# burn-research/OpenMEASURE

Measured on AMD Instinct MI355X. Metric: SPR fit+reconstruct throughput (GB/s snapshot matrix), higher is better.
Workload: dtype f64

## Files before the change

openmeasure_amd/csrc/common.hpp:

```cpp
#pragma once
#include <hip/hip_runtime.h>
#include <stdint.h>
#include <stdio.h>

#include "spr_hip.h"

typedef double f64x4 __attribute__((ext_vector_type(4)));
typedef double f64x2 __attribute__((ext_vector_type(2)));

void spr_set_error(const char *fmt, ...);

#define SPR_REQUIRE(cond, code, ...)      \
  do {                                    \
    if (!(cond)) {                        \
      spr_set_error(__VA_ARGS__);         \
      return (code);                      \
    }                                     \
  } while (0)

#define SPR_HIP_TRY(expr)                                                          \
  do {                                                                             \
    hipError_t e__ = (expr);                                                       \
    if (e__ != hipSuccess) {                                                       \
      spr_set_error("%s failed: %s (%s:%d)", #expr, hipGetErrorString(e__),       \
                    __FILE__, __LINE__);                                           \
      return SPR_E_HIP;                                                            \
    }                                                                              \
  } while (0)

#define SPR_LAUNCH_CHECK()                                                         \
  do {                                                                             \
    hipError_t e__ = hipGetLastError();                                            \
    if (e__ != hipSuccess) {                                                       \
      spr_set_error("kernel launch failed: %s (%s:%d)", hipGetErrorString(e__),   \
                    __FILE__, __LINE__);                                           \
      return SPR_E_HIP;                                                            \
    }                                                                              \
  } while (0)

int spr_cached_cus();

struct SegPlan {
  int64_t row0, n_rows, n_points;
  int32_t n_features;
  int32_t total_wg;
  int32_t chunk_rows;
};

__host__ __device__ inline void seg_range(const SegPlan &p, int f, int64_t &lo, int64_t &hi) {
  int64_t glo = (int64_t)f * p.n_points, ghi = glo + p.n_points;
  if (glo < p.row0) glo = p.row0;
  if (ghi > p.row0 + p.n_rows) ghi = p.row0 + p.n_rows;
  if (ghi < glo) ghi = glo;
  lo = glo - p.row0;
  hi = ghi - p.row0;
}

__host__ __device__ inline int seg_wgs(const SegPlan &p, int64_t rows) {
  if (rows <= 0) return 0;
  int64_t w = rows * (int64_t)p.total_wg / p.n_rows;
  int64_t chunks = (rows + p.chunk_rows - 1) / p.chunk_rows;
  if (w > chunks) w = chunks;
  if (w < 1) w = 1;
  return (int)w;
}

__host__ __device__ inline int seg_first_feature(const SegPlan &p) { return (int)(p.row0 / p.n_points); }
__host__ __device__ inline int seg_last_feature(const SegPlan &p) {
  int64_t f = (p.row0 + p.n_rows - 1) / p.n_points;
  if (f > p.n_features - 1) f = p.n_features - 1;
  return (int)f;
}

inline int seg_total_wgs(const SegPlan &p) {
  int tot = 0;
  for (int f = seg_first_feature(p); f <= seg_last_feature(p); ++f) {
    int64_t lo, hi;
    seg_range(p, f, lo, hi);
    tot += seg_wgs(p, hi - lo);
  }
  return tot;
}

__device__ inline bool seg_locate(const SegPlan &p, int b, int &f, int &wl, int &wpf, int &base,
                                  int64_t &lo, int64_t &hi) {
  int acc = 0;
  int f1 = seg_last_feature(p);
  for (int ff = seg_first_feature(p); ff <= f1; ++ff) {
    seg_range(p, ff, lo, hi);
    int w = seg_wgs(p, hi - lo);
    if (b < acc + w) {
      f = ff; wl = b - acc; wpf = w; base = acc;
      return true;
    }
    acc += w;
  }
  return false;
}

template <int CTRL>
__device__ inline double dpp_f64(double v) {
  union { double d; int i[2]; } a, b;
  a.d = v;
  b.i[0] = __builtin_amdgcn_update_dpp(0, a.i[0], CTRL, 0xF, 0xF, true);
  b.i[1] = __builtin_amdgcn_update_dpp(0, a.i[1], CTRL, 0xF, 0xF, true);
  return b.d;
}

template <int WIDTH>
__device__ inline double group_sum_t(double v) {
  if (WIDTH >= 2) v += dpp_f64<0xB1>(v);
  if (WIDTH >= 4) v += dpp_f64<0x4E>(v);
  if (WIDTH >= 8) v += dpp_f64<0x141>(v);
  if (WIDTH >= 16) v += dpp_f64<0x140>(v);
  if (WIDTH >= 32) v += __shfl_xor(v, 16, 64);
  if (WIDTH >= 64) v += __shfl_xor(v, 32, 64);
  return v;
}

__device__ inline double group_sum(double v, int width) {
  for (int o = width >> 1; o > 0; o >>= 1) v += __shfl_xor(v, o, 64);
  return v;
}

constexpr int spr_pow2_divisor_le64(int n) {
  int p = 1;
  while (p < 64 && n % (2 * p) == 0) p *= 2;
  return p;
}

inline int spr_round_mt(int m) {
  static const int sup[] = {1, 2, 3, 4, 6, 8, 12, 16};
  int need = (m + 15) / 16;
  for (int s : sup)
    if (s >= need) return s;
  return -1;
}
```

openmeasure_amd/csrc/field_dot.hpp:

```cpp
#pragma once
#include "common.hpp"

constexpr int SPR_FIELD_NF = 1;

template <int NT>
__device__ inline double field_row_value(const double (&v)[NT], const double (&a)[NT], double scale, double mean) {
  double d = 0.0;
#pragma unroll
  for (int ct = 0; ct < NT; ++ct) d = fma(v[ct], a[ct], d);
  return fma(scale, group_sum_t<16>(d), mean);
}
```

openmeasure_amd/csrc/project_ws.hip:

```cpp
#include <type_traits>

#include "rowtile.hpp"
#include "launch.hpp"
#include "project_ws.hpp"
#include "field_dot.hpp"

namespace {

constexpr int WS_WAVES = 8;
constexpr int WS_ROWS = 16 * WS_WAVES;

template <int RT> struct WsLds { static constexpr int NC = 16 * RT, LDW = NC; static_assert(RT % 2 == 0, "column tiles come in pairs"); };

template <typename TX> struct WsPiece;
template <> struct WsPiece<double> { f64x2 a, b; };
template <> struct WsPiece<float> { float x, y, z, w; };

template <int VEC, typename TX>
__device__ inline WsPiece<TX> ws_load(const TX *__restrict__ rp, int col0, int m) {
  WsPiece<TX> p;
  if constexpr (std::is_same<TX, double>::value) {
    if (VEC) {
      p.a = *reinterpret_cast<const f64x2 *>(rp + col0);
      p.b = *reinterpret_cast<const f64x2 *>(rp + col0 + 2);
    } else {
      p.a.x = rp[col0 < m ? col0 : 0];         p.a.y = rp[col0 + 1 < m ? col0 + 1 : 0];
      p.b.x = rp[col0 + 2 < m ? col0 + 2 : 0]; p.b.y = rp[col0 + 3 < m ? col0 + 3 : 0];
    }
  } else {
    if (VEC) {
      const float4 v = *reinterpret_cast<const float4 *>(rp + col0);
      p.x = v.x; p.y = v.y; p.z = v.z; p.w = v.w;
    } else {
      p.x = rp[col0 < m ? col0 : 0];         p.y = rp[col0 + 1 < m ? col0 + 1 : 0];
      p.z = rp[col0 + 2 < m ? col0 + 2 : 0]; p.w = rp[col0 + 3 < m ? col0 + 3 : 0];
    }
  }
  return p;
}

template <typename TX>
__device__ inline double ws_elem(const WsPiece<TX> &p, int t) {
  if constexpr (std::is_same<TX, double>::value) return t == 0 ? p.a.x : t == 1 ? p.a.y : t == 2 ? p.b.x : p.b.y;
  else return (double)(t == 0 ? p.x : t == 1 ? p.y : t == 2 ? p.z : p.w);
}

template <int MT, int RT, int VEC, typename TX, typename TU, bool NRM, int NF>
__global__ __launch_bounds__(WS_WAVES * 64) void project_ws_kernel(
    const TX *__restrict__ X, int64_t ldx, int m, int center_i, SegPlan plan, const double *__restrict__ inv_scale,
    const double *__restrict__ rowmean, const double *__restrict__ W, int r, TU *__restrict__ Ur, int64_t ldu,
    double *__restrict__ nrm2, WsField fld) {
  constexpr int K = 16 * MT, NJ = MT;
  constexpr int NC = WsLds<RT>::NC, LDW = WsLds<RT>::LDW;
  __shared__ double Wl[K * LDW];

  int f, wl, wpf, base;
  int64_t lo, hi;
  if (!seg_locate(plan, blockIdx.x, f, wl, wpf, base, lo, hi)) return;

  const int lane = threadIdx.x & 63;
  const int wave = __builtin_amdgcn_readfirstlane(threadIdx.x >> 6);
  const int li = lane & 15, kk = lane >> 4;
  const double isc = inv_scale[f];

  for (int e = threadIdx.x; e < K * NC; e += WS_WAVES * 64) {
    const int k = e / NC, c = e - k * NC;
    Wl[k * LDW + (c >> 5) * 32 + (c & 15) * 2 + ((c >> 4) & 1)] = (k < m && c < r) ? W[(int64_t)k * r + c] * isc : 0.0;
  }
  __syncthreads();
  double wbar[RT];
#pragma unroll
  for (int ct = 0; ct < RT; ++ct) {
    double sacc = 0.0;
    if (center_i != 0) {
      for (int k = kk; k < K; k += 4) sacc += Wl[k * LDW + (ct >> 1) * 32 + li * 2 + (ct & 1)];
      sacc += __shfl_xor(sacc, 16, 64);
      sacc += __shfl_xor(sacc, 32, 64);
    }
    wbar[ct] = sacc;
  }

  double av[NF > 0 ? NF : 1][RT];
  double fsc = 0.0;
  if constexpr (NF > 0) {
    fsc = fld.scale[f];
#pragma unroll
    for (int v = 0; v < NF; ++v)
#pragma unroll
      for (int ct = 0; ct < RT; ++ct)
        av[v][ct] = (v < fld.n_p && 16 * ct + li < r) ? fld.A[(int64_t)v * r + 16 * ct + li] : 0.0;
  }

  const int64_t nchunks = (hi - lo + WS_ROWS - 1) / WS_ROWS;
  int64_t c = wl;
  if (c >= nchunks) return;
  const double *wb = Wl + (4 * kk) * LDW + 2 * li;
  const double *wb_hi = wb + 128 * LDW;

  auto row_ptr = [&](int64_t cc) {
    int64_t row = lo + cc * WS_ROWS + 16 * wave + li;
    row = row < hi ? row : hi - 1;
    return X + row * ldx;
  };
  WsPiece<TX> areg[NJ];
  {
    const TX *rp = row_ptr(c);
#pragma unroll
    for (int j = 0; j < NJ; ++j) areg[j] = ws_load<VEC, TX>(rp, 16 * j + 4 * kk, m);
  }
  while (c < nchunks) {
    const int64_t cn = c + wpf;
    const TX *rpn = row_ptr(cn < nchunks ? cn : c);
    const int64_t blk0 = lo + c * WS_ROWS + 16 * wave;
    double mu[4];
#pragma unroll
    for (int i = 0; i < 4; ++i) {
      const int64_t rr = blk0 + kk + 4 * i;
      const double v = rowmean[rr < hi ? rr : hi - 1];
      mu[i] = center_i != 0 ? v : 0.0;
    }
    f64x4 acc[RT];
#pragma unroll
    for (int ct = 0; ct < RT; ++ct) acc[ct] = (f64x4){0.0, 0.0, 0.0, 0.0};
    f64x2 bcur[RT / 2], bnxt[RT / 2];
#pragma unroll
    for (int p = 0; p < RT / 2; ++p) bcur[p] = *reinterpret_cast<const f64x2 *>(wb + 32 * p);
#pragma unroll
    for (int j = 0; j < NJ; ++j) {
#pragma unroll
      for (int t = 0; t < 4; ++t) {
        const int sn = 4 * j + t + 1;
        const int jn = (sn >> 2) % NJ, tn = sn & 3;
        const double *wj = (jn < 8 ? wb : wb_hi) + (16 * (jn & 7) + tn) * LDW;
#pragma unroll
        for (int p = 0; p < RT / 2; ++p) bnxt[p] = *reinterpret_cast<const f64x2 *>(wj + 32 * p);
        const double a = ws_elem<TX>(areg[j], t);
#pragma unroll
        for (int p = 0; p < RT / 2; ++p) {
          acc[2 * p] = __builtin_amdgcn_mfma_f64_16x16x4f64(a, bcur[p].x, acc[2 * p], 0, 0, 0);
          acc[2 * p + 1] = __builtin_amdgcn_mfma_f64_16x16x4f64(a, bcur[p].y, acc[2 * p + 1], 0, 0, 0);
        }
        if (t == 3) areg[j] = ws_load<VEC, TX>(rpn, 16 * j + 4 * kk, m);
        __builtin_amdgcn_sched_group_barrier(0x100, RT / 2, 0);
        __builtin_amdgcn_sched_group_barrier(0x008, RT, 0);
        __builtin_amdgcn_sched_barrier(0);
#pragma unroll
        for (int p = 0; p < RT / 2; ++p) bcur[p] = bnxt[p];
      }
    }
    {
      const bool full = (blk0 + 16 <= hi) && (r == NC);
      TU *up = Ur + (blk0 + kk) * ldu + li;
      double q[4] = {0.0, 0.0, 0.0, 0.0};
      double sv[NF > 0 ? 4 : 1][RT];
#pragma unroll
      for (int ct = 0; ct < RT; ++ct) {
        const double s[4] = {acc[ct].x - mu[0] * wbar[ct], acc[ct].y - mu[1] * wbar[ct],
                             acc[ct].z - mu[2] * wbar[ct], acc[ct].w - mu[3] * wbar[ct]};
        if (NRM) {
#pragma unroll
          for (int i = 0; i < 4; ++i) { const double v = (double)(TU)s[i]; q[i] = fma(v, v, q[i]); }
        }
        if constexpr (NF > 0) {
#pragma unroll
          for (int i = 0; i < 4; ++i) sv[i][ct] = (double)(TU)s[i];
        }
        if (full) {
#pragma unroll
          for (int i = 0; i < 4; ++i) up[4 * i * ldu + 16 * ct] = (TU)s[i];
        } else if (16 * ct + li < r) {
#pragma unroll
          for (int i = 0; i < 4; ++i)
            if (blk0 + kk + 4 * i < hi) up[4 * i * ldu + 16 * ct] = (TU)s[i];
        }
      }
      if (NRM) {
#pragma unroll
        for (int i = 0; i < 4; ++i) {
          const double t = group_sum_t<16>(q[i]);
          if (li == i && blk0 + kk + 4 * i < hi) nrm2[blk0 + kk + 4 * i] = t;
        }
      }
      if constexpr (NF > 0) {
#pragma unroll
        for (int v = 0; v < NF; ++v)
#pragma unroll
          for (int i = 0; i < 4; ++i) {
            const double x = field_row_value<RT>(sv[i], av[v], fsc, mu[i]);
            if (li == i && v < fld.n_p && blk0 + kk + 4 * i < hi) fld.out[(int64_t)v * fld.ldo + blk0 + kk + 4 * i] = x;
          }
      }
    }
    c = cn;
  }
}

template <int MT, int RT, typename TX, typename TU>
int ws_launch(const TX *X, int64_t n_rows, int32_t m, int64_t ldx, int64_t row0, int64_t n_points, int32_t n_features,
              int center, const double *inv_scale, const double *rowmean, const double *W, int32_t r, TU *Ur,
              int64_t ldu, int accumulate, double *nrm2, hipStream_t st, const WsField *field) {
  SegPlan plan = spr_make_plan(row0, n_rows, n_points, n_features, WS_ROWS);
  constexpr int narrow_per_cu = 2;
  const int grid = spr_plan_grid(plan, MT <= 4 ? narrow_per_cu : 1);
  const bool vec = (m == 16 * MT) && spr_rows_aligned16(X, sizeof(TX) * ldx);
  if (!vec) return SPR_E_UNSUPPORTED;
  const WsField fld = field ? *field : WsField{nullptr, nullptr, 0, nullptr, 0};
#define WS_GO(NRMV, NFV)                                                                                                       \
  hipLaunchKernelGGL((project_ws_kernel<MT, RT, 1, TX, TU, NRMV, NFV>), dim3(grid), dim3(WS_WAVES * 64), 0, st, X, ldx, (int)m, \
                     center, plan, inv_scale, rowmean, W, (int)r, Ur, ldu, nrm2, fld)
  if (field) {
    if (nrm2) WS_GO(true, SPR_FIELD_NF);
    else WS_GO(false, SPR_FIELD_NF);
  } else {
    if (nrm2) WS_GO(true, 0);
    else WS_GO(false, 0);
  }
#undef WS_GO
  SPR_LAUNCH_CHECK();
  return SPR_OK;
}

}


template <typename TX, typename TU>
int spr_project_ws(const TX *d_X, int64_t n_rows, int32_t m, int64_t ldx, int64_t row0, int64_t n_points,
                   int32_t n_features, int32_t center, const double *d_inv_scale, const double *d_rowmean,
                   const double *d_W, int32_t r, TU *d_Ur, int64_t ldu, int32_t accumulate, double *d_rownorm2,
                   hipStream_t st, const WsField *field) {
  if (accumulate) return SPR_E_UNSUPPORTED;
  if (field && (field->n_p < 1 || field->n_p > SPR_FIELD_NF || r % 16 != 0 || !center)) return SPR_E_UNSUPPORTED;
  const int mt = spr_round_mt(m);
  const int need = (r + 15) / 16;
  const int rt = need <= 2 ? 2 : need <= 4 ? 4 : 0;
#define WS(MTV, RTV)                                                                                             \
  if (mt == MTV && rt == RTV)                                                                                    \
    return ws_launch<MTV, RTV, TX, TU>(d_X, n_rows, m, ldx, row0, n_points, n_features, center, d_inv_scale,   \
                                        d_rowmean, d_W, r, d_Ur, ldu, accumulate, d_rownorm2, st, field)
  WS(4, 2); WS(4, 4); WS(8, 2); WS(8, 4); WS(12, 2); WS(12, 4); WS(16, 2); WS(16, 4);
#undef WS
  return SPR_E_UNSUPPORTED;
}

template int spr_project_ws<double, double>(const double *, int64_t, int32_t, int64_t, int64_t, int64_t, int32_t, int32_t,
                                            const double *, const double *, const double *, int32_t, double *, int64_t,
                                            int32_t, double *, hipStream_t, const WsField *);
template int spr_project_ws<float, float>(const float *, int64_t, int32_t, int64_t, int64_t, int64_t, int32_t, int32_t,
                                          const double *, const double *, const double *, int32_t, float *, int64_t,
                                          int32_t, double *, hipStream_t, const WsField *);
template int spr_project_ws<float, double>(const float *, int64_t, int32_t, int64_t, int64_t, int64_t, int32_t, int32_t,
                                           const double *, const double *, const double *, int32_t, double *, int64_t,
                                           int32_t, double *, hipStream_t, const WsField *);
```

openmeasure_amd/csrc/rowtile.hpp:

```cpp
#pragma once
#include "common.hpp"

typedef float f32x2 __attribute__((ext_vector_type(2)));
template <typename TX> struct PieceOf;
template <> struct PieceOf<double> { using type = f64x2; };
template <> struct PieceOf<float> { using type = f32x2; };
__device__ inline f64x2 widen(f64x2 p) { return p; }
__device__ inline f64x2 widen(f32x2 p) { return (f64x2){(double)p.x, (double)p.y}; }

struct RowStats {
  double cnt, ref, s1, s2;
  __device__ inline void init() { cnt = 0.0; ref = 0.0; s1 = 0.0; s2 = 0.0; }
  __device__ inline void push(double x, bool valid) {
    ref = (cnt == 0.0) ? x : ref;
    const double d = valid ? x - ref : 0.0;
    cnt += valid ? 1.0 : 0.0;
    s1 += d;
    s2 += d * d;
  }
  __device__ inline double mean() const { return cnt > 0.0 ? ref + s1 / cnt : 0.0; }
  __device__ inline double m2() const {
    const double v = cnt > 0.0 ? s2 - s1 * s1 / cnt : 0.0;
    return v > 0.0 ? v : 0.0;
  }
// ... 13 lines not shown
  static_assert(R % ROWS_PER_IT == 0, "panel rows must be a multiple of rows per pass");
  static constexpr bool WIDE_STORE = (MP % 2 == 0);

  Piece pre[IT][VPL];
  double pmean[IT];

  template <int VEC>
  __device__ inline void load_pass(int it, const TX *__restrict__ X, int64_t ldx, int m, int64_t crow0,
                                   int64_t seg_hi, int wave, int lane, const double *__restrict__ mean_in = nullptr,
                                   int split = 1 << 30, int64_t gap = 0) {
    const int grp = lane / LPR, lig = lane % LPR;
    int64_t lrow = crow0 + it * ROWS_PER_IT + wave * RPW + grp;
    lrow = lrow < seg_hi ? lrow : seg_hi - 1;
    const TX *rp = X + lrow * ldx;
    if (mean_in) pmean[it] = mean_in[lrow];
#pragma unroll
    for (int v = 0; v < VPL; ++v) {
      const int col = 2 * (lig + v * LPR);
      const int64_t g0 = col >= split ? gap : 0, g1 = col + 1 >= split ? gap : 0;
      Piece t;
      if (VEC == 2) {
        t = *reinterpret_cast<const Piece *>(rp + col + g0);
      } else if (VEC == 1) {
        t = *reinterpret_cast<const Piece *>(rp + (col < m ? col + g0 : 0));
      } else {
        t.x = rp[col < m ? col + g0 : 0];
        t.y = rp[col + 1 < m ? col + 1 + g1 : 0];
      }
      pre[it][v] = t;
    }
  }

  template <int VEC>
  __device__ inline void load_piece(int it, int v, const TX *__restrict__ X, int64_t ldx, int m, int64_t crow0,
                                    int64_t seg_hi, int wave, int lane) {
    const int grp = lane / LPR, lig = lane % LPR;
    int64_t lrow = crow0 + it * ROWS_PER_IT + wave * RPW + grp;
    lrow = lrow < seg_hi ? lrow : seg_hi - 1;
    const TX *rp = X + lrow * ldx;
    const int col = 2 * (lig + v * LPR);
    Piece t;
    if (VEC == 2) {
      t = *reinterpret_cast<const Piece *>(rp + col);
    } else if (VEC == 1) {
      t = *reinterpret_cast<const Piece *>(rp + (col < m ? col : 0));
    } else {
      t.x = rp[col < m ? col : 0];
      t.y = rp[col + 1 < m ? col + 1 : 0];
    }
    pre[it][v] = t;
  }

  __device__ inline void raw_store_piece(int it, int v, double *__restrict__ lds, int m, int64_t crow0,
                                         int64_t seg_hi, int wave, int lane) {
    const int grp = lane / LPR, lig = lane % LPR;
    const int rloc = it * ROWS_PER_IT + wave * RPW + grp;
    const bool rv = crow0 + rloc < seg_hi;
    const int col = 2 * (lig + v * LPR);
    f64x2 c = widen(pre[it][v]);
    c.x = (rv && col < m) ? c.x : 0.0;
    c.y = (rv && col + 1 < m) ? c.y : 0.0;
    if constexpr (WIDE_STORE) {
      *reinterpret_cast<f64x2 *>(lds + rloc * MP + col) = c;
    } else {
      lds[rloc * MP + col] = c.x;
      lds[rloc * MP + col + 1] = c.y;
    }
  }

  template <int VEC>
  __device__ inline void load(const TX *__restrict__ X, int64_t ldx, int m, int64_t crow0, int64_t seg_hi,
                              int wave, int lane, const double *__restrict__ mean_in = nullptr, int split = 1 << 30,
                              int64_t gap = 0) {
#pragma unroll
    for (int it = 0; it < IT; ++it) load_pass<VEC>(it, X, ldx, m, crow0, seg_hi, wave, lane, mean_in, split, gap);
  }

  template <bool WRITE_MEAN>
  __device__ inline void center_store_pass(int it, double *__restrict__ lds, int m, int center, int64_t crow0,
                                           int64_t seg_hi, int wave, int lane, double *__restrict__ rowmean,
                                           RowStats *st, double *__restrict__ rowsum = nullptr) {
    const int grp = lane / LPR, lig = lane % LPR;
    const double inv_m = 1.0 / (double)m;
    const int rloc = it * ROWS_PER_IT + wave * RPW + grp;
    const int64_t lrow = crow0 + rloc;
    const bool rv = lrow < seg_hi;
    const bool fast = (crow0 + (it + 1) * ROWS_PER_IT <= seg_hi) && (m == MPAD);
    if (fast) {
      double mean;
      if constexpr (WRITE_MEAN) {
        double s = 0.0;
#pragma unroll
        for (int v = 0; v < VPL; ++v) { const f64x2 w = widen(pre[it][v]); s += w.x + w.y; }
        s = group_sum_t<LPR>(s);
        mean = center == 2 ? pmean[it] : (center ? s * inv_m : 0.0);
        if (rowsum && center == 2 && lig == 0) rowsum[lrow] = s;
      } else {
        mean = center ? pmean[it] : 0.0;
      }
      if (WRITE_MEAN) {
        if (lig == 0 && center != 2) rowmean[lrow] = mean;
        st->push(mean, center != 2);
      }
#pragma unroll
      for (int v = 0; v < VPL; ++v) {
        const int col = 2 * (lig + v * LPR);
        const f64x2 w = widen(pre[it][v]);
        f64x2 c = {w.x - mean, w.y - mean};
        if constexpr (WIDE_STORE) {
          *reinterpret_cast<f64x2 *>(lds + rloc * MP + col) = c;
        } else {
          lds[rloc * MP + col] = c.x;
          lds[rloc * MP + col + 1] = c.y;
        }
      }
      return;
    }
    double s = 0.0;
#pragma unroll
    for (int v = 0; v < VPL; ++v) {
      const int col = 2 * (lig + v * LPR);
      const f64x2 w = widen(pre[it][v]);
      s += (col < m ? w.x : 0.0) + (col + 1 < m ? w.y : 0.0);
    }
    s = group_sum_t<LPR>(s);
    const double mean = center == 2 ? pmean[it] : (center ? s * inv_m : 0.0);
    if (WRITE_MEAN) {
      if (rv && lig == 0 && center != 2) rowmean[lrow] = mean;
      if (rowsum && center == 2 && rv && lig == 0) rowsum[lrow] = s;
      st->push(mean, rv && center != 2);
    }
#pragma unroll
    for (int v = 0; v < VPL; ++v) {
      const int col = 2 * (lig + v * LPR);
      const f64x2 w = widen(pre[it][v]);
      f64x2 c;
      c.x = (rv && col < m) ? w.x - mean : 0.0;
      c.y = (rv && col + 1 < m) ? w.y - mean : 0.0;
      if constexpr (WIDE_STORE) {
        *reinterpret_cast<f64x2 *>(lds + rloc * MP + col) = c;
      } else {
        lds[rloc * MP + col] = c.x;
        lds[rloc * MP + col + 1] = c.y;
      }
    }
  }

  template <bool EXT>
  __device__ inline void load_pass_own(int it, const TX *__restrict__ ubase, int64_t ldx, int64_t lane_off,
                                       int64_t rows_left, int wave, int lane, const double *__restrict__ mean_in,
                                       int64_t crow0, int split = 1 << 30, int64_t gap = 0) {
    const int grp = lane / LPR, lig = lane % LPR;
    const int64_t lrow = (int64_t)it * ROWS_PER_IT + wave * RPW + grp;
    const int64_t last = rows_left > 0 ? rows_left - 1 : 0;
    const bool in = lrow < rows_left;
    const int64_t off = in ? lane_off + (int64_t)it * ROWS_PER_IT * ldx : last * ldx;
    const TX *rp = ubase + off;
    if (EXT) pmean[it] = mean_in[crow0 + (in ? lrow : last)];
#pragma unroll
    for (int v = 0; v < VPL; ++v) {
      const int col = 2 * (lig + v * LPR);
      pre[it][v] = *reinterpret_cast<const Piece *>(rp + col + (col >= split ? gap : 0));
    }
  }

  template <bool FULL, bool EXT, bool SUMS = false>
  __device__ inline void center_store_own(int it, double *__restrict__ lds, int64_t crow0, int64_t rows_left, int wave,
                                          int lane, double *__restrict__ rowmean, double *__restrict__ rowsum = nullptr) {
    const int grp = lane / LPR, lig = lane % LPR;
    constexpr double inv_m = 1.0 / (double)MPAD;
    const int rloc = it * ROWS_PER_IT + wave * RPW + grp;
    const bool rv = FULL || rloc < rows_left;
    f64x2 w[VPL];
#pragma unroll
    for (int v = 0; v < VPL; ++v) w[v] = widen(pre[it][v]);
    double mean;
    if (EXT) {
      mean = pmean[it];
      if (SUMS) {
        double s = w[0].x + w[0].y;
#pragma unroll
        for (int v = 1; v < VPL; ++v) s += w[v].x + w[v].y;
        s = group_sum_t<LPR>(s);
        if (rv && lig == 0) rowsum[crow0 + rloc] = s;
      }
    } else {
      double s = w[0].x + w[0].y;
#pragma unroll
      for (int v = 1; v < VPL; ++v) s += w[v].x + w[v].y;
      s = group_sum_t<LPR>(s);
      mean = s * inv_m;
      if (rv && lig == 0) rowmean[crow0 + rloc] = mean;
    }
#pragma unroll
    for (int v = 0; v < VPL; ++v) {
      const int col = 2 * (lig + v * LPR);
      f64x2 c = {w[v].x - mean, w[v].y - mean};
      if (!FULL) {
        c.x = rv ? c.x : 0.0;
        c.y = rv ? c.y : 0.0;
      }
      *reinterpret_cast<f64x2 *>(lds + rloc * MP + col) = c;
    }
  }

  __device__ inline void raw_store_pass(int it, double *__restrict__ lds, int m, int64_t crow0, int64_t seg_hi,
                                        int wave, int lane) {
    const int grp = lane / LPR, lig = lane % LPR;
    const int rloc = it * ROWS_PER_IT + wave * RPW + grp;
    const bool rv = crow0 + rloc < seg_hi;
    const bool fast = (crow0 + (it + 1) * ROWS_PER_IT <= seg_hi) && (m == MPAD);
#pragma unroll
    for (int v = 0; v < VPL; ++v) {
      const int col = 2 * (lig + v * LPR);
      f64x2 c = widen(pre[it][v]);
      if (!fast) {
        c.x = (rv && col < m) ? c.x : 0.0;
        c.y = (rv && col + 1 < m) ? c.y : 0.0;
      }
      if constexpr (WIDE_STORE) {
        *reinterpret_cast<f64x2 *>(lds + rloc * MP + col) = c;
      } else {
        lds[rloc * MP + col] = c.x;
        lds[rloc * MP + col + 1] = c.y;
      }
    }
  }

  __device__ inline void raw_store(double *__restrict__ lds, int m, int64_t crow0, int64_t seg_hi, int wave,
                                   int lane) {
#pragma unroll
    for (int it = 0; it < IT; ++it) raw_store_pass(it, lds, m, crow0, seg_hi, wave, lane);
  }

  template <bool WRITE_MEAN>
  __device__ inline void center_store(double *__restrict__ lds, int m, int center, int64_t crow0, int64_t seg_hi,
                                      int wave, int lane, double *__restrict__ rowmean, RowStats *st,
                                      double *__restrict__ rowsum = nullptr) {
#pragma unroll
    for (int it = 0; it < IT; ++it)
      center_store_pass<WRITE_MEAN>(it, lds, m, center, crow0, seg_hi, wave, lane, rowmean, st, rowsum);
  }
};
```

openmeasure_amd/csrc/stats_gram.hip:

```cpp
#include <type_traits>

#include "rowtile.hpp"
#include "launch.hpp"

#define GRAM_MFMA(a, b, c) __builtin_amdgcn_mfma_f64_16x16x4f64((a), (b), (c), 0, 0, 0)

namespace {

template <int MT>
struct GramShape {
  static constexpr int MPAD = 16 * MT;
  static constexpr int MP = MPAD + ((MT % 2 == 0) ? 16 : 0);
  static constexpr int T = MT * (MT + 1) / 2;
  static constexpr int NU = (MT + 1) / 2;
};

template <int MT> struct GramCfg;
template <> struct GramCfg<1>  { static constexpr int NW = 8,  R = 64, KS = 8; static constexpr bool DBUF = true; static constexpr int LPRMAX = 16; };
template <> struct GramCfg<2>  { static constexpr int NW = 8,  R = 32, KS = 8; static constexpr bool DBUF = true; static constexpr int LPRMAX = 16; };
template <> struct GramCfg<3>  { static constexpr int NW = 8,  R = 64, KS = 4; static constexpr bool DBUF = true; static constexpr int LPRMAX = 16; };
template <> struct GramCfg<4>  { static constexpr int NW = 8,  R = 64, KS = 4; static constexpr bool DBUF = true; static constexpr int LPRMAX = 8; };
template <> struct GramCfg<6>  { static constexpr int NW = 12, R = 48, KS = 4; static constexpr bool DBUF = true; static constexpr int LPRMAX = 16; };
template <> struct GramCfg<8>  { static constexpr int NW = 8,  R = 32, KS = 2; static constexpr bool DBUF = true; static constexpr int LPRMAX = 16; };
template <> struct GramCfg<12> { static constexpr int NW = 12, R = 24, KS = 2; static constexpr bool DBUF = false; static constexpr int LPRMAX = 32; };
template <> struct GramCfg<16> { static constexpr int NW = 8,  R = 32, KS = 1; static constexpr bool DBUF = false; static constexpr int LPRMAX = 16; };

template <int MT> struct GramOut { static constexpr int KSO = (GramCfg<MT>::KS >= 4) ? 1 : GramCfg<MT>::KS; };

constexpr int tri_index(int mt, int ti, int tj) { return ti * mt - ti * (ti - 1) / 2 + (tj - ti); }

template <int MT>
__device__ inline void tile_coords(int idx, int &ti, int &tj) {
  ti = 0;
  while (ti < MT - 1 && idx >= MT - ti) { idx -= MT - ti; ++ti; }
  tj = ti + idx;
  if (tj > MT - 1) tj = MT - 1;
}

template <int MT, int U, int VEC, typename TX>
__device__ inline void gram_wave(const TX *__restrict__ X, int64_t ldx, int m, int center,
                                 int64_t lo, int64_t hi, int wl, int wpf, int ks, int wave, int lane,
                                 double *__restrict__ lds0, double *__restrict__ lds1,
                                 double *__restrict__ rowmean, double *__restrict__ stat_part,
                                 double *__restrict__ slab, double *__restrict__ rowsum) {
  using S = GramShape<MT>;
  using C = GramCfg<MT>;
  constexpr int R = C::R, KS = C::KS, NW = C::NW, MP = S::MP, T = S::T;
  constexpr int KROWS = R / KS, KSTEPS = KROWS / 4;
  constexpr int RA = U, RB = MT - 1 - U;
  constexpr int NA = MT - RA;
  constexpr int NB = (RB != RA) ? MT - RB : 0;
  static_assert(KROWS % 4 == 0, "k slice must be a multiple of the MFMA depth");
  using RT = RowTile<MT, R, MP, NW, C::LPRMAX, TX>;

  f64x4 accA[NA];
  f64x4 accB[NB > 0 ? NB : 1];
#pragma unroll
  for (int j = 0; j < NA; ++j) accA[j] = (f64x4){0.0, 0.0, 0.0, 0.0};
#pragma unroll
  for (int j = 0; j < NB; ++j) accB[j] = (f64x4){0.0, 0.0, 0.0, 0.0};

  RowStats st;
  st.init();
  RT tile;

  const int64_t nchunks = (hi - lo + R - 1) / R;
  int64_t c = wl;
  const double *mean_in = rowmean;
  tile.template load<VEC>(X, ldx, m, lo + c * R, hi, wave, lane, mean_in);
  tile.template center_store<true>(lds0, m, center, lo + c * R, hi, wave, lane, rowmean, &st, rowsum);
  int64_t cn = c + wpf;
  int64_t nrow0 = (cn < nchunks) ? lo + cn * R : hi;
  tile.template load<VEC>(X, ldx, m, nrow0, hi, wave, lane, mean_in);
  int buf = 0;
  const int frag = (lane >> 4) * MP + (lane & 15) + ks * KROWS * MP + RA * 16;
  while (c < nchunks) {
    double *cur = buf ? lds1 : lds0;
    double *nxt = buf ? lds0 : lds1;
    const int64_t c2 = cn + wpf;
    const int64_t n2row0 = (c2 < nchunks) ? lo + c2 * R : hi;
    __syncthreads();
    const double *p = cur + frag;
    if constexpr (C::DBUF) {
      double op[2][NA];
#pragma unroll
      for (int j = 0; j < NA; ++j) op[0][j] = p[16 * j];
#pragma unroll
      for (int k = 0; k < KSTEPS; ++k) {
        if (k + 1 < KSTEPS) {
#pragma unroll
          for (int j = 0; j < NA; ++j) op[(k + 1) & 1][j] = p[(k + 1) * 4 * MP + 16 * j];
        }
#pragma unroll
        for (int j = 0; j < NA; ++j)
          accA[j] = GRAM_MFMA(op[k & 1][0], op[k & 1][j], accA[j]);
#pragma unroll
        for (int j = 0; j < NB; ++j)
          accB[j] = GRAM_MFMA(op[k & 1][RB - RA], op[k & 1][RB - RA + j], accB[j]);
#pragma unroll
        for (int it = 0; it < RT::IT; ++it)
          if ((it * KSTEPS) / RT::IT == k) {
            tile.template center_store_pass<true>(it, nxt, m, center, nrow0, hi, wave, lane, rowmean, &st, rowsum);
            tile.template load_pass<VEC>(it, X, ldx, m, n2row0, hi, wave, lane, mean_in);
          }
      }
    } else {
#pragma unroll
      for (int k = 0; k < KSTEPS; ++k) {
        double op[NA];
#pragma unroll
        for (int j = 0; j < NA; ++j) op[j] = p[k * 4 * MP + 16 * j];
#pragma unroll
        for (int j = 0; j < NA; ++j)
          accA[j] = GRAM_MFMA(op[0], op[j], accA[j]);
#pragma unroll
        for (int j = 0; j < NB; ++j)
          accB[j] = GRAM_MFMA(op[RB - RA], op[RB - RA + j], accB[j]);
#pragma unroll
        for (int it = 0; it < RT::IT; ++it)
          if ((it * KSTEPS) / RT::IT == k) {
            tile.template center_store_pass<true>(it, nxt, m, center, nrow0, hi, wave, lane, rowmean, &st, rowsum);
            tile.template load_pass<VEC>(it, X, ldx, m, n2row0, hi, wave, lane, mean_in);
          }
      }
    }
    buf ^= 1;
    c = cn;
    cn = c2;
    nrow0 = n2row0;
  }

  constexpr int KSO = GramOut<MT>::KSO;
  if constexpr (KSO != KS) {
    static_assert((size_t)T * 256 <= (size_t)2 * R * MP, "tile staging must fit the panel buffers");
    double *red = lds0 + lane;
    for (int s = KS - 1; s >= 1; --s) {
      __syncthreads();
      if (ks == s) {
#pragma unroll
        for (int j = 0; j < NA; ++j) {
          double *tp = red + tri_index(MT, RA, RA + j) * 256;
          tp[0] = accA[j].x; tp[64] = accA[j].y; tp[128] = accA[j].z; tp[192] = accA[j].w;
        }
#pragma unroll
        for (int j = 0; j < NB; ++j) {
          double *tp = red + tri_index(MT, RB, RB + j) * 256;
          tp[0] = accB[j].x; tp[64] = accB[j].y; tp[128] = accB[j].z; tp[192] = accB[j].w;
        }
      }
      __syncthreads();
      if (ks == s - 1) {
#pragma unroll
        for (int j = 0; j < NA; ++j) {
          const double *tp = red + tri_index(MT, RA, RA + j) * 256;
          accA[j].x += tp[0]; accA[j].y += tp[64]; accA[j].z += tp[128]; accA[j].w += tp[192];
        }
#pragma unroll
        for (int j = 0; j < NB; ++j) {
          const double *tp = red + tri_index(MT, RB, RB + j) * 256;
          accB[j].x += tp[0]; accB[j].y += tp[64]; accB[j].z += tp[128]; accB[j].w += tp[192];
        }
      }
    }
  }
  if (KSO == KS || ks == 0) {
    double *sp = slab + ((int64_t)blockIdx.x * KSO + (KSO == KS ? ks : 0)) * T * 256 + lane;
#pragma unroll
    for (int j = 0; j < NA; ++j) {
      double *tp = sp + (int64_t)tri_index(MT, RA, RA + j) * 256;
      tp[0] = accA[j].x; tp[64] = accA[j].y; tp[128] = accA[j].z; tp[192] = accA[j].w;
    }
#pragma unroll
    for (int j = 0; j < NB; ++j) {
      double *tp = sp + (int64_t)tri_index(MT, RB, RB + j) * 256;
      tp[0] = accB[j].x; tp[64] = accB[j].y; tp[128] = accB[j].z; tp[192] = accB[j].w;
    }
  }
  if ((lane % RT::LPR) == 0) {
    double *q = stat_part + ((int64_t)blockIdx.x * RT::ROWS_PER_IT + wave * RT::RPW + lane / RT::LPR) * 3;
    q[0] = st.cnt; q[1] = st.mean(); q[2] = st.m2();
  }
}

__device__ inline void chan_merge(double &n, double &mu, double &m2, double nb, double mb, double sb) {
  if (nb > 0.0) {
    const double tot = n + nb, d = mb - mu;
    mu += d * nb / tot;
    m2 += sb + d * d * n * nb / tot;
    n = tot;
  }
}

template <int MT, int U, typename TX, bool EXT, bool SUMS>
__device__ inline void gram_wave_own(const TX *__restrict__ X, int64_t ldx, int64_t lo, int64_t hi, int wl, int wpf, int ks,
                                     int wave, int lane, double *__restrict__ lds0, double *__restrict__ lds1,
                                     double *__restrict__ rowmean, double *__restrict__ slab, double *__restrict__ rowsum) {
  using S = GramShape<MT>;
  using C = GramCfg<MT>;
  constexpr int R = C::R, KS = C::KS, NW = C::NW, MP = S::MP, T = S::T;
  constexpr int KROWS = R / KS, KSTEPS = KROWS / 4;
  constexpr int RA = U, RB = MT - 1 - U;
  constexpr int NA = MT - RA;
  constexpr int NB = (RB != RA) ? MT - RB : 0;
  using RT = RowTile<MT, R, MP, NW, C::LPRMAX, TX>;

  f64x4 accA[NA];
  f64x4 accB[NB > 0 ? NB : 1];
#pragma unroll
  for (int j = 0; j < NA; ++j) accA[j] = (f64x4){0.0, 0.0, 0.0, 0.0};
#pragma unroll
  for (int j = 0; j < NB; ++j) accB[j] = (f64x4){0.0, 0.0, 0.0, 0.0};

  RT tile;
  const int64_t nchunks = (hi - lo + R - 1) / R;
  const int64_t lane_off = (int64_t)(wave * RT::RPW + lane / RT::LPR) * ldx;
  auto base_of = [&](int64_t row0) { return X + row0 * ldx; };
  int64_t c = wl;
  int64_t crow0 = lo + c * R;
#pragma unroll
  for (int it = 0; it < RT::IT; ++it) tile.template load_pass_own<EXT>(it, base_of(crow0), ldx, lane_off, hi - crow0, wave, lane, rowmean, crow0);
  if (crow0 + R <= hi) {
#pragma unroll
    for (int it = 0; it < RT::IT; ++it) tile.template center_store_own<true, EXT, SUMS>(it, lds0, crow0, hi - crow0, wave, lane, rowmean, rowsum);
  } else {
#pragma unroll
    for (int it = 0; it < RT::IT; ++it) tile.template center_store_own<false, EXT, SUMS>(it, lds0, crow0, hi - crow0, wave, lane, rowmean, rowsum);
  }
  int64_t cn = c + wpf;
  int64_t nrow0 = (cn < nchunks) ? lo + cn * R : hi;
#pragma unroll
  for (int it = 0; it < RT::IT; ++it) tile.template load_pass_own<EXT>(it, base_of(nrow0 < hi ? nrow0 : lo), ldx, lane_off, hi - nrow0, wave, lane, rowmean, nrow0 < hi ? nrow0 : lo);
  int buf = 0;
  const int frag = (lane >> 4) * MP + (lane & 15) + ks * KROWS * MP + RA * 16;
  while (c < nchunks) {
    double *cur = buf ? lds1 : lds0;
    double *nxt = buf ? lds0 : lds1;
    const int64_t c2 = cn + wpf;
    const int64_t n2row0 = (c2 < nchunks) ? lo + c2 * R : hi;
    const TX *n2base = base_of(n2row0 < hi ? n2row0 : lo);
    const bool nfull = nrow0 + R <= hi;
    __syncthreads();
    const double *p = cur + frag;
    auto stage = [&](auto full_tag, int k) {
      constexpr bool FULL = decltype(full_tag)::value;
#pragma unroll
      for (int it = 0; it < RT::IT; ++it)
        if ((it * KSTEPS) / RT::IT == k) {
          tile.template center_store_own<FULL, EXT, SUMS>(it, nxt, nrow0, hi - nrow0, wave, lane, rowmean, rowsum);
          tile.template load_pass_own<EXT>(it, n2base, ldx, lane_off, hi - n2row0, wave, lane, rowmean, n2row0 < hi ? n2row0 : lo);
        }
    };
    if constexpr (C::DBUF) {
      double op[2][NA];
#pragma unroll
      for (int j = 0; j < NA; ++j) op[0][j] = p[16 * j];
#pragma unroll
      for (int k = 0; k < KSTEPS; ++k) {
        if (k + 1 < KSTEPS) {
#pragma unroll
          for (int j = 0; j < NA; ++j) op[(k + 1) & 1][j] = p[(k + 1) * 4 * MP + 16 * j];
        }
#pragma unroll
        for (int j = 0; j < NA; ++j) accA[j] = GRAM_MFMA(op[k & 1][0], op[k & 1][j], accA[j]);
#pragma unroll
        for (int j = 0; j < NB; ++j) accB[j] = GRAM_MFMA(op[k & 1][RB - RA], op[k & 1][RB - RA + j], accB[j]);
        if (nfull) stage(std::true_type{}, k); else stage(std::false_type{}, k);
      }
    } else {
#pragma unroll
      for (int k = 0; k < KSTEPS; ++k) {
        double op[NA];
#pragma unroll
        for (int j = 0; j < NA; ++j) op[j] = p[k * 4 * MP + 16 * j];
#pragma unroll
        for (int j = 0; j < NA; ++j) accA[j] = GRAM_MFMA(op[0], op[j], accA[j]);
#pragma unroll
        for (int j = 0; j < NB; ++j) accB[j] = GRAM_MFMA(op[RB - RA], op[RB - RA + j], accB[j]);
        if (nfull) stage(std::true_type{}, k); else stage(std::false_type{}, k);
      }
    }
    buf ^= 1;
    c = cn;
    cn = c2;
    nrow0 = n2row0;
  }
  double *sp = slab + ((int64_t)blockIdx.x * KS + ks) * T * 256 + lane;
#pragma unroll
  for (int j = 0; j < NA; ++j) {
    double *tp = sp + (int64_t)tri_index(MT, RA, RA + j) * 256;
    tp[0] = accA[j].x; tp[64] = accA[j].y; tp[128] = accA[j].z; tp[192] = accA[j].w;
  }
#pragma unroll
  for (int j = 0; j < NB; ++j) {
    double *tp = sp + (int64_t)tri_index(MT, RB, RB + j) * 256;
    tp[0] = accB[j].x; tp[64] = accB[j].y; tp[128] = accB[j].z; tp[192] = accB[j].w;
  }
}

template <int MT, typename TX, bool EXT, bool SUMS>
__global__ __launch_bounds__(GramCfg<MT>::NW * 64) void stats_gram_own_kernel(
    const TX *__restrict__ X, int64_t ldx, SegPlan plan, double *__restrict__ rowmean, double *__restrict__ slab,
    double *__restrict__ rowsum) {
  using S = GramShape<MT>;
  using C = GramCfg<MT>;
  constexpr int NU = S::NU;
  __shared__ double lds[2][C::R * S::MP];
  int f, wl, wpf, base;
  int64_t lo, hi;
  if (!seg_locate(plan, blockIdx.x, f, wl, wpf, base, lo, hi)) return;
  const int lane = threadIdx.x & 63;
  const int wave = __builtin_amdgcn_readfirstlane(threadIdx.x >> 6);
  const int ks = wave / NU;
  const int unit = (NU == 8 && C::KS == 1) ? ((wave < 4) ? wave : 11 - wave) : wave % NU;
#define GRAM_UNIT(UV)                                                                                          \
  case UV:                                                                                                     \
    if constexpr (UV < NU)                                                                                     \
      gram_wave_own<MT, UV, TX, EXT, SUMS>(X, ldx, lo, hi, wl, wpf, ks, wave, lane, lds[0], lds[1], rowmean, slab, rowsum); \
    break;
  switch (unit) {
    GRAM_UNIT(0) GRAM_UNIT(1) GRAM_UNIT(2) GRAM_UNIT(3) GRAM_UNIT(4) GRAM_UNIT(5) GRAM_UNIT(6) GRAM_UNIT(7)
    default: break;
  }
#undef GRAM_UNIT
}

constexpr int RS_THREADS = 1024;
__global__ __launch_bounds__(RS_THREADS) void gram_rowmean_stats_kernel(const double *__restrict__ rowmean, SegPlan plan,
                                                                        int slots_per_wg, double *__restrict__ stat_part) {
  __shared__ double sn[RS_THREADS / 64], smu[RS_THREADS / 64], sm2[RS_THREADS / 64];
  int f, wl, wpf, base;
  int64_t lo, hi;
  if (!seg_locate(plan, blockIdx.x, f, wl, wpf, base, lo, hi)) return;
  const int lane = threadIdx.x & 63, wave = threadIdx.x >> 6;
  RowStats st;
  st.init();
  const int64_t step = (int64_t)wpf * RS_THREADS;
  int64_t row = lo + (int64_t)wl * RS_THREADS + threadIdx.x;
  for (; row + 3 * step < hi; row += 4 * step) {
    const double a = rowmean[row], b = rowmean[row + step], c = rowmean[row + 2 * step], d = rowmean[row + 3 * step];
    st.push(a, true); st.push(b, true); st.push(c, true); st.push(d, true);
  }
  for (; row < hi; row += step) st.push(rowmean[row], true);
  double n = st.cnt, mu = st.mean(), m2 = st.m2();
  for (int o = 32; o > 0; o >>= 1) {
    const double on = __shfl_down(n, o, 64), om = __shfl_down(mu, o, 64), os = __shfl_down(m2, o, 64);
    chan_merge(n, mu, m2, on, om, os);
  }
  if (lane == 0) { sn[wave] = n; smu[wave] = mu; sm2[wave] = m2; }
  __syncthreads();
  double *q = stat_part + (int64_t)blockIdx.x * slots_per_wg * 3;
  if (threadIdx.x == 0) {
    n = 0.0; mu = 0.0; m2 = 0.0;
    for (int w = 0; w < RS_THREADS / 64; ++w) chan_merge(n, mu, m2, sn[w], smu[w], sm2[w]);
    q[0] = n; q[1] = mu; q[2] = m2;
  }
  for (int e = 3 + threadIdx.x; e < slots_per_wg * 3; e += RS_THREADS) q[e] = 0.0;
}

template <int MT, int VEC, typename TX>
__global__ __launch_bounds__(GramCfg<MT>::NW * 64) void stats_gram_kernel(
    const TX *__restrict__ X, int64_t ldx, int m, int center_i, SegPlan plan,
    double *__restrict__ rowmean, double *__restrict__ stat_part, double *__restrict__ slab, double *__restrict__ rowsum) {
  using S = GramShape<MT>;
  using C = GramCfg<MT>;
  constexpr int NU = S::NU;
  static_assert(NU * C::KS == C::NW, "waves = units x k slices");
  __shared__ double lds[2][C::R * S::MP];

  int f, wl, wpf, base;
  int64_t lo, hi;
  if (!seg_locate(plan, blockIdx.x, f, wl, wpf, base, lo, hi)) return;

  const int lane = threadIdx.x & 63;
  const int wave = __builtin_amdgcn_readfirstlane(threadIdx.x >> 6);
  const int unit = wave % NU, ks = wave / NU;
#define GRAM_UNIT(UV)                                                                                        \
  case UV:                                                                                                   \
    if constexpr (UV < NU)                                                                                   \
      gram_wave<MT, UV, VEC, TX>(X, ldx, m, center_i, lo, hi, wl, wpf, ks, wave, lane, lds[0],    \
                        lds[1], rowmean, stat_part, slab, rowsum);                                           \
    break;
  switch (unit) {
    GRAM_UNIT(0) GRAM_UNIT(1) GRAM_UNIT(2) GRAM_UNIT(3) GRAM_UNIT(4) GRAM_UNIT(5) GRAM_UNIT(6) GRAM_UNIT(7)
    default: break;
  }
#undef GRAM_UNIT
}

template <int MT>
__global__ __launch_bounds__(1024) void gram_finalize_kernel(
    const double *__restrict__ slab, const double *__restrict__ stat_part, int m, SegPlan plan,
    int slots_per_wg, double *__restrict__ gram, double *__restrict__ fstats, int ldg, int origin) {
  constexpr int T = GramShape<MT>::T;
  constexpr int KS = GramOut<MT>::KSO;
  __shared__ double red[4][256];
  const int f = blockIdx.y;
  const int tile = blockIdx.x;
  int base = 0, wpf = 0;
  {
    int acc = 0;
    const int f0 = seg_first_feature(plan), f1 = seg_last_feature(plan);
    for (int ff = f0; ff <= f1; ++ff) {
      int64_t lo, hi;
      seg_range(plan, ff, lo, hi);
      const int w = seg_wgs(plan, hi - lo);
      if (ff == f) { base = acc; wpf = w; }
      acc += w;
    }
  }
  int ti, tj;
  tile_coords<MT>(tile, ti, tj);
  const int e = threadIdx.x & 255, g = threadIdx.x >> 8;
  const int np = wpf * KS;
  const double *sp = slab + ((int64_t)base * KS * T + tile) * 256 + e;
  const int64_t stride = (int64_t)T * 256;
  double s0 = 0.0, s1 = 0.0, s2 = 0.0, s3 = 0.0;
  int p = g;
  for (; p + 12 < np; p += 16) {
    s0 += sp[p * stride];
    s1 += sp[(p + 4) * stride];
    s2 += sp[(p + 8) * stride];
// ... 243 lines not shown
```

Baseline: 1231.

## Cut per-row reduction and bounds overhead in projection and Gram kernels

The projection kernel now reduces four row values in one combined DPP butterfly (group_sum4_t) instead of four separate 16-lane reductions, for both the norms and the field reconstruction. It also replaces 64-bit row clamping with a uniform per-block row limit and a scalar offset, and adds a fast store path when the U matrix is packed. The Gram kernel and row tile loader use a scalar-forced 64-bit compare (uniform_lt) to keep branch conditions in SGPRs, and mark LDS operand loads volatile in the non-double-buffered path. The aim is fewer VALU and DPP instructions and less register pressure, at the cost of inline asm that constrains the compiler and more complex lane-to-slot mapping logic.

```diff
diff --git a/openmeasure_amd/csrc/common.hpp b/openmeasure_amd/csrc/common.hpp
--- a/openmeasure_amd/csrc/common.hpp
+++ b/openmeasure_amd/csrc/common.hpp
@@ -98,6 +98,12 @@
   return false;
 }
 
+__device__ inline bool uniform_lt(int64_t a, int64_t b) {
+  int d_hi = (int)(((uint64_t)a - (uint64_t)b) >> 32);
+  asm("" : "+s"(d_hi));
+  return d_hi < 0;
+}
+
 template <int CTRL>
 __device__ inline double dpp_f64(double v) {
   union { double d; int i[2]; } a, b;
@@ -118,6 +124,19 @@
   return v;
 }
 
+__device__ inline int group_sum4_slot(int li) { return (li ^ ((li & 4) ? 3 : 0)) & 3; }
+
+__device__ inline double group_sum4_t(double v0, double v1, double v2, double v3, int li) {
+  const int slot = group_sum4_slot(li);
+  const bool odd = slot & 1, up = slot & 2;
+  const double a0 = (odd ? v1 : v0) + dpp_f64<0xB1>(odd ? v0 : v1);
+  const double a1 = (odd ? v3 : v2) + dpp_f64<0xB1>(odd ? v2 : v3);
+  double s = (up ? a1 : a0) + dpp_f64<0x4E>(up ? a0 : a1);
+  s += dpp_f64<0x141>(s);
+  s += dpp_f64<0x140>(s);
+  return s;
+}
+
 __device__ inline double group_sum(double v, int width) {
   for (int o = width >> 1; o > 0; o >>= 1) v += __shfl_xor(v, o, 64);
   return v;
diff --git a/openmeasure_amd/csrc/field_dot.hpp b/openmeasure_amd/csrc/field_dot.hpp
--- a/openmeasure_amd/csrc/field_dot.hpp
+++ b/openmeasure_amd/csrc/field_dot.hpp
@@ -10,3 +10,17 @@
   for (int ct = 0; ct < NT; ++ct) d = fma(v[ct], a[ct], d);
   return fma(scale, group_sum_t<16>(d), mean);
 }
+
+template <int NT>
+__device__ inline double field_row4_value(const double (&v)[4][NT], const double (&a)[NT], double scale, double mean0,
+                                          double mean1, double mean2, double mean3, int li) {
+  double d0 = 0.0, d1 = 0.0, d2 = 0.0, d3 = 0.0;
+#pragma unroll
+  for (int ct = 0; ct < NT; ++ct) {
+    d0 = fma(v[0][ct], a[ct], d0); d1 = fma(v[1][ct], a[ct], d1);
+    d2 = fma(v[2][ct], a[ct], d2); d3 = fma(v[3][ct], a[ct], d3);
+  }
+  const int slot = group_sum4_slot(li);
+  const double mu_lo = (slot & 1) ? mean1 : mean0, mu_hi = (slot & 1) ? mean3 : mean2;
+  return fma(scale, group_sum4_t(d0, d1, d2, d3, li), (slot & 2) ? mu_hi : mu_lo);
+}
diff --git a/openmeasure_amd/csrc/project_ws.hip b/openmeasure_amd/csrc/project_ws.hip
--- a/openmeasure_amd/csrc/project_ws.hip
+++ b/openmeasure_amd/csrc/project_ws.hip
@@ -95,13 +95,24 @@
   int64_t c = wl;
   if (c >= nchunks) return;
   const double *wb = Wl + (4 * kk) * LDW + 2 * li;
-  const double *wb_hi = wb + 128 * LDW;
-
+  int hi_off = 128 * LDW;
+  if constexpr (NJ > 8) asm volatile("" : "+v"(hi_off));
+  const double *wb_hi = wb + hi_off;
+
+  auto row_lim = [&](int64_t blk0) {
+    const uint64_t e = (uint64_t)(hi - 1 - blk0 + WS_ROWS);
+    const uint32_t e_lo = (uint32_t)e, e_hi = (uint32_t)(e >> 32), top = WS_ROWS + 15;
+    return (int)(e_hi ? top : (e_lo < top ? e_lo : top)) - WS_ROWS;
+  };
+  const int64_t lrow = (int64_t)li * ldx;
   auto row_ptr = [&](int64_t cc) {
-    int64_t row = lo + cc * WS_ROWS + 16 * wave + li;
-    row = row < hi ? row : hi - 1;
-    return X + row * ldx;
+    const int64_t blk0 = lo + cc * WS_ROWS + 16 * wave;
+    const int lim = row_lim(blk0);
+    int64_t limrow = lim * ldx;
+    asm volatile("" : "+s"(limrow));
+    return X + blk0 * ldx + (li <= lim ? lrow : limrow);
   };
+  const bool packed = (r == NC) && (ldu == NC);
   WsPiece<TX> areg[NJ];
   {
     const TX *rp = row_ptr(c);
@@ -112,12 +123,17 @@
     const int64_t cn = c + wpf;
     const TX *rpn = row_ptr(cn < nchunks ? cn : c);
     const int64_t blk0 = lo + c * WS_ROWS + 16 * wave;
+    const int lim = row_lim(blk0);
     double mu[4];
-#pragma unroll
-    for (int i = 0; i < 4; ++i) {
-      const int64_t rr = blk0 + kk + 4 * i;
-      const double v = rowmean[rr < hi ? rr : hi - 1];
-      mu[i] = center_i != 0 ? v : 0.0;
+    {
+      const char *mp = reinterpret_cast<const char *>(rowmean + (lim < 0 ? hi - 1 : blk0));
+      const uint32_t lim8 = lim < 0 ? 0u : 8u * lim;
+#pragma unroll
+      for (int i = 0; i < 4; ++i) {
+        const uint32_t o8 = 8u * (kk + 4 * i);
+        const double v = *reinterpret_cast<const double *>(mp + (o8 < lim8 ? o8 : lim8));
+        mu[i] = center_i != 0 ? v : 0.0;
+      }
     }
     f64x4 acc[RT];
 #pragma unroll
@@ -149,46 +165,51 @@
       }
     }
     {
-      const bool full = (blk0 + 16 <= hi) && (r == NC);
-      TU *up = Ur + (blk0 + kk) * ldu + li;
+      const bool full = (lim == 15) && (r == NC);
       double q[4] = {0.0, 0.0, 0.0, 0.0};
-      double sv[NF > 0 ? 4 : 1][RT];
+      double sv[4][RT];
 #pragma unroll
       for (int ct = 0; ct < RT; ++ct) {
         const double s[4] = {acc[ct].x - mu[0] * wbar[ct], acc[ct].y - mu[1] * wbar[ct],
                              acc[ct].z - mu[2] * wbar[ct], acc[ct].w - mu[3] * wbar[ct]};
-        if (NRM) {
-#pragma unroll
-          for (int i = 0; i < 4; ++i) { const double v = (double)(TU)s[i]; q[i] = fma(v, v, q[i]); }
-        }
-        if constexpr (NF > 0) {
-#pragma unroll
-          for (int i = 0; i < 4; ++i) sv[i][ct] = (double)(TU)s[i];
-        }
-        if (full) {
-#pragma unroll
-          for (int i = 0; i < 4; ++i) up[4 * i * ldu + 16 * ct] = (TU)s[i];
-        } else if (16 * ct + li < r) {
-#pragma unroll
-          for (int i = 0; i < 4; ++i)
-            if (blk0 + kk + 4 * i < hi) up[4 * i * ldu + 16 * ct] = (TU)s[i];
-        }
-      }
+#pragma unroll
+        for (int i = 0; i < 4; ++i) {
+          sv[i][ct] = (double)(TU)s[i];
+          if (NRM) q[i] = fma(sv[i][ct], sv[i][ct], q[i]);
+        }
+      }
+      if (full && packed) {
+        TU *up = Ur + blk0 * NC + (kk * NC + li);
+#pragma unroll
+        for (int ct = 0; ct < RT; ++ct)
+#pragma unroll
+          for (int i = 0; i < 4; ++i) up[4 * i * NC + 16 * ct] = (TU)sv[i][ct];
+      } else {
+        TU *up = Ur + (blk0 + kk) * ldu + li;
+#pragma unroll
+        for (int ct = 0; ct < RT; ++ct) {
+          if (full) {
+#pragma unroll
+            for (int i = 0; i < 4; ++i) up[4 * i * ldu + 16 * ct] = (TU)sv[i][ct];
+          } else if (16 * ct + li < r) {
+#pragma unroll
+            for (int i = 0; i < 4; ++i)
+              if (kk + 4 * i <= lim) up[4 * i * ldu + 16 * ct] = (TU)sv[i][ct];
+          }
+        }
+      }
+      const int orow = kk + 4 * li;
+      const bool writer = li < 4 && orow <= lim;
       if (NRM) {
-#pragma unroll
-        for (int i = 0; i < 4; ++i) {
-          const double t = group_sum_t<16>(q[i]);
-          if (li == i && blk0 + kk + 4 * i < hi) nrm2[blk0 + kk + 4 * i] = t;
-        }
+        const double t = group_sum4_t(q[0], q[1], q[2], q[3], li);
+        if (writer) nrm2[blk0 + orow] = t;
       }
       if constexpr (NF > 0) {
 #pragma unroll
-        for (int v = 0; v < NF; ++v)
-#pragma unroll
-          for (int i = 0; i < 4; ++i) {
-            const double x = field_row_value<RT>(sv[i], av[v], fsc, mu[i]);
-            if (li == i && v < fld.n_p && blk0 + kk + 4 * i < hi) fld.out[(int64_t)v * fld.ldo + blk0 + kk + 4 * i] = x;
-          }
+        for (int v = 0; v < NF; ++v) {
+          const double x = field_row4_value<RT>(sv, av[v], fsc, mu[0], mu[1], mu[2], mu[3], li);
+          if (writer && v < fld.n_p) fld.out[(int64_t)v * fld.ldo + blk0 + orow] = x;
+        }
       }
     }
     c = cn;
diff --git a/openmeasure_amd/csrc/rowtile.hpp b/openmeasure_amd/csrc/rowtile.hpp
--- a/openmeasure_amd/csrc/rowtile.hpp
+++ b/openmeasure_amd/csrc/rowtile.hpp
@@ -189,8 +189,15 @@
                                        int64_t crow0, int split = 1 << 30, int64_t gap = 0) {
     const int grp = lane / LPR, lig = lane % LPR;
     const int64_t lrow = (int64_t)it * ROWS_PER_IT + wave * RPW + grp;
-    const int64_t last = rows_left > 0 ? rows_left - 1 : 0;
-    const bool in = lrow < rows_left;
+    int64_t last;
+    bool in;
+    if constexpr (!EXT) {
+      last = uniform_lt(0, rows_left) ? rows_left - 1 : 0;
+      in = (int)lrow < (uniform_lt(rows_left, R) ? (int)rows_left : R);
+    } else {
+      last = rows_left > 0 ? rows_left - 1 : 0;
+      in = lrow < rows_left;
+    }
     const int64_t off = in ? lane_off + (int64_t)it * ROWS_PER_IT * ldx : last * ldx;
     const TX *rp = ubase + off;
     if (EXT) pmean[it] = mean_in[crow0 + (in ? lrow : last)];
diff --git a/openmeasure_amd/csrc/stats_gram.hip b/openmeasure_amd/csrc/stats_gram.hip
--- a/openmeasure_amd/csrc/stats_gram.hip
+++ b/openmeasure_amd/csrc/stats_gram.hip
@@ -6,6 +6,8 @@
 #define GRAM_MFMA(a, b, c) __builtin_amdgcn_mfma_f64_16x16x4f64((a), (b), (c), 0, 0, 0)
 
 namespace {
+
+typedef volatile __attribute__((address_space(3))) double lds_operand_t;
 
 template <int MT>
 struct GramShape {
@@ -236,21 +238,22 @@
     double *cur = buf ? lds1 : lds0;
     double *nxt = buf ? lds0 : lds1;
     const int64_t c2 = cn + wpf;
-    const int64_t n2row0 = (c2 < nchunks) ? lo + c2 * R : hi;
-    const TX *n2base = base_of(n2row0 < hi ? n2row0 : lo);
-    const bool nfull = nrow0 + R <= hi;
+    const bool more = uniform_lt(c2, nchunks);
+    const int64_t n2row0 = more ? lo + c2 * R : hi;
+    const TX *n2base = base_of(more ? n2row0 : lo);
+    const bool nfull = !uniform_lt(hi, nrow0 + R);
     __syncthreads();
-    const double *p = cur + frag;
     auto stage = [&](auto full_tag, int k) {
       constexpr bool FULL = decltype(full_tag)::value;
 #pragma unroll
       for (int it = 0; it < RT::IT; ++it)
         if ((it * KSTEPS) / RT::IT == k) {
           tile.template center_store_own<FULL, EXT, SUMS>(it, nxt, nrow0, hi - nrow0, wave, lane, rowmean, rowsum);
-          tile.template load_pass_own<EXT>(it, n2base, ldx, lane_off, hi - n2row0, wave, lane, rowmean, n2row0 < hi ? n2row0 : lo);
+          tile.template load_pass_own<EXT>(it, n2base, ldx, lane_off, hi - n2row0, wave, lane, rowmean, more ? n2row0 : lo);
         }
     };
     if constexpr (C::DBUF) {
+      const double *p = cur + frag;
       double op[2][NA];
 #pragma unroll
       for (int j = 0; j < NA; ++j) op[0][j] = p[16 * j];
@@ -267,6 +270,7 @@
         if (nfull) stage(std::true_type{}, k); else stage(std::false_type{}, k);
       }
     } else {
+      const lds_operand_t *p = (const lds_operand_t *)(cur + frag);
 #pragma unroll
       for (int k = 0; k < KSTEPS; ++k) {
         double op[NA];
```

Measured after the change: 1263, median of 6. +2.6%, better.
